# robin-karlsson0/pc-accumulation-lib

Measured on AMD Instinct MI355X. Metric: Mpoints/s projected+accumulated and BEV frames/s @256x256; 1/2/4/8 GPU, higher is better.
Workload: dtype f64; 1 GPU; KITTI-360 single forward cam, 120k pts/frame, 200 m horizon (~201 live frames, 5169634 stored pts), one 256x256x21 BEV per integrated frame; points_per_frame=120000, bev_px=256, view_m=80

## Files before the change

### include/pca.h

```cpp
#ifndef PCA_H
#define PCA_H

#include <stdint.h>

#ifdef __cplusplus
extern "C" {
#endif

#define PCA_VERSION 2

typedef struct pca_ctx pca_ctx;

typedef struct {
    double *x, *y, *z;
    float *intensity;
    uint32_t *rgbs;
    int32_t *inst;
    uint8_t *dyn;
    int64_t capacity;
    uint32_t *frame_box;
} pca_store;

#define PCA_STATUS_STORE_OVERFLOW 1u
#define PCA_STATUS_UV_OUT_OF_IMAGE 2u
// ... 322 lines not shown

typedef struct pca_host_track pca_host_track;
typedef struct {
    const void *pts;
    const void *rgb;
    const void *sem;
    const void *sem_gt;
    int32_t n;
    uint32_t host_mask;
} pca_kitti_obs;
int pca_kitti_integrate(pca_ctx *ctx, const pca_kitti_obs *obs, const double P[12], int H, int W,
                        const uint64_t filter_mask[4], const pca_store *store, int64_t *frame_off , int slot,
                        int sample_mode, pca_host_track *track, const double *T_new_prev, double horizon, int64_t *evicted,
                        double *path_length, void *stream);
void pca_host_camera_cone(const double P[12], int H, int W, double cone[15]);
int pca_host_view_hull(int F, const double *then , const float *box , const double *cone ,
                       const double now[12], const pca_bev_params *prm, int *first, int *last);
int pca_bev_bin_range(pca_ctx *ctx, int slot_first, int slot_last_plus1);
int pca_bev_view_hint(pca_ctx *ctx, int slot0, int F, const double *then, const float *box, const double *cone, const double now[12],
                      const pca_bev_params *prm);
void pca_f32_box_decode(const uint32_t *rows , int n, float *box );

int pca_debug_bev_level1(const pca_ctx *ctx, int out[4]);
int pca_debug_icp_layout(int32_t n_src, int32_t n_tgt, int64_t out[16]);

int pca_k1_defer(pca_ctx *ctx, int on);
int pca_k1_flush(pca_ctx *ctx);
int pca_kitti_generate_bev(pca_ctx *ctx, const pca_store *store, const int64_t *frame_off , int slot_begin,
                           int slot_split, int slot_end, int64_t max_points, const pca_bev_params *prm,
                           const double *pending_Ts, const int *pending_slot_ends, int n_pending, int write_back,
                           void *workspace , int64_t workspace_bytes, uint16_t *planes_f16 ,
                           void *host_planes , const pca_host_track *track, double *traj_rows,
                           int32_t *traj_start, int32_t *n_rows, void *stream);

typedef struct {
    const pca_kitti_obs *obs; const double *P; int32_t H, W; const uint64_t *filter_mask; const pca_store *store;
    int64_t *frame_off; int32_t slot, sample_mode; pca_host_track *track; const double *T_new_prev; double horizon;
    int64_t evicted; double path_length; void *stream;
} pca_kitti_integrate_args;
int pca_kitti_integrate_v(pca_ctx *ctx, pca_kitti_integrate_args *a);
typedef struct {
    const pca_store *store; const int64_t *frame_off; int32_t slot_begin, slot_split, slot_end, pad0; int64_t max_points;
    const pca_bev_params *prm; const double *pending_Ts; const int *pending_slot_ends; int32_t n_pending, write_back;
    void *workspace; int64_t workspace_bytes; uint16_t *planes_f16; void *host_planes; const pca_host_track *track;
    double *traj_rows; int32_t *traj_start; int32_t n_rows, pad1; void *stream;
    int32_t hint_slot0, hint_F; const double *hint_then; const float *hint_box; const double *hint_cone; const double *hint_now;
// ... 88 lines not shown
```

### pc-accumulation-lib_amd/csrc/pca_bev.hip

```cpp
#include "pca_bev_common.h"
#include "pca_bev_view.h"
#include "pca_k1_body.h"
#include <cstdlib>
#include <mutex>

#define NFK (2 * TCELLS)
#ifndef AB_THREADS
#define AB_THREADS 1024
#endif
#define MAX_G 512
#ifndef BIN_RUNR
#define BIN_RUNR 4
#endif
#ifndef BIN_WPE
#define BIN_WPE 4
#endif
#ifndef BIN_UNR
#define BIN_UNR 4
#endif
#ifndef BIN_REG_P
#define BIN_REG_P 12
#endif
#ifndef C_THREADS
#define C_THREADS 256
#endif
#define C_WAVES (C_THREADS / 64)
#define C_HIST_WAVES 4
#define RGB_CAP 4096
#ifndef C_SLOT_Q
#define C_SLOT_Q 4
#endif
#define CONTIG_MIN 2560
#define HEAVY_MIN_DEFAULT 2560
#define FLAG_ROAD (1u << 24)
#define FLAG_DYNOBJ (1u << 25)

struct __attribute__((aligned(16))) RecF { double z; uint32_t iw; uint32_t cw; };
struct RecD { double z; double inten; uint32_t c; uint32_t fk; };

struct alignas(16) BevArgs {
    pca_store st;
    const double *intensity64;
    const int64_t *frame_off;
    int slot_begin, slot_split, slot_end;
// ... 6 lines not shown
    int heavy_min;
    int stagger;
    uint32_t *key;
    uint32_t *bh;
    uint32_t *boff;
    int Gk;
    int bin_first, bin_end;
    int k1_slot, k1_n;
    uint32_t *bh0;
    int split;
    uint32_t *heavy_hint;
    uint32_t heavy_hint_known;
    uint32_t *span_hint;
    uint32_t span_hint_known;
    int heavy_launched;
    uint32_t *heavy;
    void *recs;
    double *planes;
    uint16_t *planes_f16;
    double *extra;
    uint32_t *status;
    int dbg;
    int band_r0, band_rows;
};
#define HQ_CLASSES 32
#define HQ_CURSOR 32
#define HQ_IDS 64

struct Window { int64_t lo, hi, sp, c_lo, c_hi; };

#define K1_SEG 4096
#define K1_RIDE 32
__device__ __forceinline__ int64_t window_end(const BevArgs &a)
{
    const int e = a.Gk ? a.k1_slot : a.slot_end;
    return a.frame_off[a.bin_end < e ? a.bin_end : e];
}
__device__ __forceinline__ int64_t window_begin(const BevArgs &a) { return a.frame_off[a.bin_first]; }
__device__ __forceinline__ Window chunk_of(const BevArgs &a, int &g)
{
    Window w;
    w.lo = window_begin(a);
    const int64_t hi0 = window_end(a);
    w.sp = (a.Gk && a.slot_split > a.k1_slot) ? hi0 : a.frame_off[a.slot_split];
    w.hi = (hi0 - w.lo > a.max_points) ? w.lo + a.max_points : hi0;
    const int G = a.G - a.Gk;
// ... 102 lines not shown
        s_dyn[threadIdx.x] = w;
    }
    BIN_STAMP(0);
    int g;
    const Window w = chunk_of(a, g);
    const int64_t chunk = seg_stride(w.hi - w.lo, a.G - a.Gk);
    const bool split = bev_split(a, w.hi - w.lo);
    const int hs = split ? 6 : 7;
    const int n_hist = split ? 2 * a.T : a.T;
    uint32_t *s_cur = s_lds + n_hist;
    if ((int)blockIdx.x == a.Gk) {
        const int64_t end_ub = a.Gk ? a.frame_off[a.k1_slot] + a.k1_n : a.frame_off[a.slot_end];
        if (threadIdx.x == 0 && end_ub - a.frame_off[a.slot_begin] > a.max_points + a.k1_n) pca_raise(a.status, PCA_STATUS_STORE_OVERFLOW);
        if (threadIdx.x < HQ_IDS) a.heavy[threadIdx.x] = 0;
        if (threadIdx.x == 0 && a.span_hint) {
            const uint32_t kp = (uint32_t)((w.hi - w.lo + 1023) >> 10);
            if (kp != a.span_hint_known) *a.span_hint = kp;
        }
    }
    for (int t = threadIdx.x; t < n_hist; t += AB_THREADS) s_h[t] = 0;
    __syncthreads();
    const PendHi pend_hi = owed_bounds(a.owed, a.frame_off, a.slot_begin, w.lo);
    const int64_t reg_hi = w.c_lo + (int64_t)REG_P * AB_THREADS < w.c_hi ? w.c_lo + (int64_t)REG_P * AB_THREADS : w.c_hi;
    uint32_t rkey[REG_P > 0 ? REG_P : 1], rrgb[REG_P > 0 ? REG_P : 1];
    float rinten[REG_P > 0 ? REG_P : 1];
    double rz[REG_P > 0 ? REG_P : 1];
    const uint32_t n_reg = w.c_lo < reg_hi ? (uint32_t)(reg_hi - w.c_lo) : 0u;
    auto rel = [&](int64_t p) -> uint32_t {
        const int64_t d = p - w.c_lo;
        return d <= 0 ? 0u : (d < (int64_t)n_reg ? (uint32_t)d : n_reg);
    };
    const uint32_t sp_rel = rel(w.sp);
    if (REG_P > 0 && n_reg > 0) {
        const double *xb = a.st.x + w.c_lo, *yb = a.st.y + w.c_lo, *zb = a.st.z + w.c_lo;
        const uint8_t *db = a.st.dyn + w.c_lo;
        const ViewConst vc = view_const(a.prm, a.tx, a.band_r0, a.band_rows);
        double XA[UNR], YA[UNR], ZA[UNR];
        uint32_t DA[UNR];
        auto issue = [&](int j0, double (&X)[UNR], double (&Y)[UNR], double (&Z)[UNR], uint32_t (&D)[UNR]) {
#pragma unroll
            for (int u = 0; u < UNR; ++u) {
                const uint32_t i = (uint32_t)(j0 + u) * AB_THREADS + threadIdx.x, ic = i < n_reg ? i : 0u;
                X[u] = xb[ic];
                Y[u] = yb[ic];
                Z[u] = zb[ic];
                D[u] = db[ic];
            }
        };
        auto work = [&](int j0, double (&X)[UNR], double (&Y)[UNR], double (&Z)[UNR], uint32_t (&D)[UNR]) {
            uint32_t n_moved = 0;
#pragma unroll 1
            for (int k = 0; k < a.owed.n_pend; ++k) {
                const Mat34 &Tk = a.owed.pend_T[k];
                const uint32_t n_owe = rel(k == 0 ? pend_hi.v[0] : k == 1 ? pend_hi.v[1] : k == 2 ? pend_hi.v[2] : pend_hi.v[3]);
                if (n_owe == 0) continue;
                n_moved = n_owe > n_moved ? n_owe : n_moved;
                const double t0 = Tk.m[0], t1 = Tk.m[1], t2 = Tk.m[2], t3 = Tk.m[3], t4 = Tk.m[4], t5 = Tk.m[5], t6 = Tk.m[6],
                             t7 = Tk.m[7], t8 = Tk.m[8], t9 = Tk.m[9], t10 = Tk.m[10], t11 = Tk.m[11];
                const uint32_t batch_end = (uint32_t)(j0 + UNR) * AB_THREADS < n_reg ? (uint32_t)(j0 + UNR) * AB_THREADS : n_reg;
                const bool all_owe = n_owe >= batch_end;
                if (all_owe) {
#pragma unroll
                    for (int u = 0; u < UNR; ++u) {
                        const double nx = fma(t2, Z[u], fma(t1, Y[u], t0 * X[u])) + t3;
                        const double ny = fma(t6, Z[u], fma(t5, Y[u], t4 * X[u])) + t7;
                        const double nz = fma(t10, Z[u], fma(t9, Y[u], t8 * X[u])) + t11;
                        X[u] = nx; Y[u] = ny; Z[u] = nz;
                    }
                } else {
#pragma unroll
                    for (int u = 0; u < UNR; ++u) {
                        const uint32_t i = (uint32_t)(j0 + u) * AB_THREADS + threadIdx.x;
                        const bool owed = i < n_owe;
                        const double nx = fma(t2, Z[u], fma(t1, Y[u], t0 * X[u])) + t3;
                        const double ny = fma(t6, Z[u], fma(t5, Y[u], t4 * X[u])) + t7;
                        const double nz = fma(t10, Z[u], fma(t9, Y[u], t8 * X[u])) + t11;
                        X[u] = owed ? nx : X[u]; Y[u] = owed ? ny : Y[u]; Z[u] = owed ? nz : Z[u];
                    }
                }
            }
            if (a.owed.write_back && n_moved > 0) {
                double *xw = a.st.x + w.c_lo, *yw = a.st.y + w.c_lo, *zw = a.st.z + w.c_lo;
#pragma unroll
                for (int u = 0; u < UNR; ++u) {
                    const uint32_t i = (uint32_t)(j0 + u) * AB_THREADS + threadIdx.x;
                    if (i < n_moved) { xw[i] = X[u]; yw[i] = Y[u]; zw[i] = Z[u]; }
                }
            }
#pragma unroll
            for (int u = 0; u < UNR; ++u) {
                const uint32_t i = (uint32_t)(j0 + u) * AB_THREADS + threadIdx.x;
                rkey[j0 + u] = view_key_lean<BAND>(vc, X[u], Y[u], Z[u], i < n_reg && D[u] != 1u, i >= sp_rel ? 1u : 0u);
                rz[j0 + u] = Z[u];
                if (rkey[j0 + u] != KEY_INVALID) atomicAdd(&s_h[rkey[j0 + u] >> hs], 1u);
            }
        };
#pragma unroll
        for (int j0 = 0; j0 < REG_P; j0 += UNR) {
            issue(j0, XA, YA, ZA, DA);
            work(j0, XA, YA, ZA, DA);
        }
    } else {
#pragma unroll
        for (int j = 0; j < REG_P; ++j) { rkey[j] = KEY_INVALID; rz[j] = 0.0; }
    }
    BIN_STAMP(1);
    constexpr int MUNR = BIN_UNR;
    const ViewConst vcm = view_const(a.prm, a.tx, a.band_r0, a.band_rows);
    for (int64_t base = reg_hi + threadIdx.x; base < w.c_hi; base += MUNR * AB_THREADS) {
        double X[MUNR], Y[MUNR], Z[MUNR];
        uint8_t D[MUNR];
#pragma unroll
        for (int u = 0; u < MUNR; ++u) {
            const int64_t p = base + u * AB_THREADS;
            const bool in = p < w.c_hi;
            X[u] = in ? a.st.x[p] : 0.0;
            Y[u] = in ? a.st.y[p] : 0.0;
            Z[u] = in ? a.st.z[p] : 0.0;
            D[u] = in ? a.st.dyn[p] : (uint8_t)1;
        }
#pragma unroll
        for (int u = 0; u < MUNR; ++u) {
            const int64_t p = base + u * AB_THREADS;
            if (p >= w.c_hi) continue;
            const BinPoint b = bin_point<BAND>(a, vcm, w, pend_hi, p, X[u], Y[u], Z[u], D[u]);
            if (b.key != KEY_INVALID) atomicAdd(&s_h[b.key >> hs], 1u);
            a.key[p - w.lo] = b.key;
        }
    }
    __syncthreads();
    BIN_STAMP(2);
    bin_scan_tables(a, s_h, s_cur, s_wsum, split, g);
// ... 1 lines not shown
    BIN_STAMP(3);
    const uint32_t seg = (uint32_t)((int64_t)a.Gk * K1_SEG + (int64_t)(g - a.Gk) * chunk);
    if (REG_P > 0 && n_reg > 0) {
        const uint32_t *cb = a.st.rgbs + w.c_lo;
        const float *ib = a.st.intensity + w.c_lo;
#pragma unroll
        for (int j = 0; j < REG_P; ++j) {
            const uint32_t i = (uint32_t)j * AB_THREADS + threadIdx.x, ic = rkey[j] != KEY_INVALID ? i : 0u;
            rrgb[j] = cb[ic];
            rinten[j] = ib[ic];
        }
        {
            uint32_t touch = 0;
#pragma unroll
            for (int j = 0; j < REG_P; ++j) touch |= rrgb[j] ^ __float_as_uint(rinten[j]);
            asm volatile("" ::"v"(touch));
        }
#pragma unroll
        for (int j = 0; j < REG_P; ++j) {
            if (rkey[j] == KEY_INVALID) continue;
            const uint32_t pos = seg + atomicAdd(&s_cur[rkey[j] >> hs], 1u);
            bin_store<I64>(a, s_dyn, pos, rkey[j], rrgb[j], rz[j], 0.0, rinten[j]);
        }
    }
    BIN_STAMP(4);
    const bool stale = a.owed.n_pend > 0 && !a.owed.write_back;
    for (int64_t base = reg_hi + threadIdx.x; base < w.c_hi; base += MUNR * AB_THREADS) {
        uint32_t key[MUNR], pos[MUNR], rgbs[MUNR];
        double zz[MUNR], iv[MUNR], xs[MUNR], ys[MUNR];
#pragma unroll
        for (int u = 0; u < MUNR; ++u) {
            const int64_t p = base + u * AB_THREADS;
            key[u] = p < w.c_hi ? a.key[p - w.lo] : KEY_INVALID;
        }
#pragma unroll
        for (int u = 0; u < MUNR; ++u) {
            const int64_t p = base + u * AB_THREADS;
            const bool ok = key[u] != KEY_INVALID;
            rgbs[u] = ok ? a.st.rgbs[p] : 0u;
            zz[u] = ok ? a.st.z[p] : 0.0;
            xs[u] = (ok && stale) ? a.st.x[p] : 0.0;
            ys[u] = (ok && stale) ? a.st.y[p] : 0.0;
            if (I64) iv[u] = ok ? a.intensity64[p] : 0.0;
            else iv[u] = ok ? (double)a.st.intensity[p] : 0.0;
        }
#pragma unroll
        for (int u = 0; u < MUNR; ++u) {
            const int64_t p = base + u * AB_THREADS;
            const bool ok = key[u] != KEY_INVALID;
            if (ok && stale) apply_owed(a.owed, pend_hi, p, xs[u], ys[u], zz[u]);
// ... 998 lines not shown
static inline int n_groups(int64_t max_points)
{
    const int max_g = max_groups(), per_g = (int)pca_env_int("PCA_BEV_CHUNK", 8192, 1024);
    int64_t g = (max_points + per_g - 1) / per_g;
    return (int)(g < 1 ? 1 : (g > max_g ? max_g : g));
}

struct BevLayout { int T, G; int64_t bh, boff, bh0, heavy, recs, total; };
static BevLayout bev_layout(int64_t max_points, int px)
{
    if (max_points < 1) max_points = 1;
    const int64_t T = (int64_t)band_rows(px) * tiles_x(px), G = n_groups(max_points);
    const int64_t table = pca_align256((G + K1_RIDE + 8) * T * 4);
    BevLayout l;
    l.T = (int)T; l.G = (int)G;
    l.bh = pca_align256(max_points * 4);
    l.boff = l.bh + table; l.bh0 = l.boff + table;
    l.heavy = l.bh0 + table;
    l.recs = l.heavy + pca_align256((HQ_IDS + HQ_CLASSES * T) * 4);
    l.total = l.recs + pca_align256((max_points + G + K1_RIDE + K1_SEG) * 24) + 512;
    return l;
}

typedef void (*BevKernel)(BevArgs);
typedef void (*BevManyKernel)();
struct BevKernelSet {
    BevKernel bin, cells, heavy[2][2];
    BevManyKernel bin_many, cells_many, heavy_many;
    int bin_lds;
};
#define K1_RIDE_LDS (80 * 1024)
#define BEV_WHOLE_SET(I)                                                                                                          \
    { bev_tile_bin<I>, bev_tile_cells<I>,                                                                                         \
      {{bev_tile_cells_heavy<I, false, false>, bev_tile_cells_heavy<I, false, true>}, {bev_tile_cells_heavy<I, true, false>, bev_tile_cells_heavy<I, true, true>}}, \
      bev_tile_bin_many<I>, bev_tile_cells_many<I>, bev_tile_cells_heavy_many<I>, 128 * 1024 }
#define BEV_BAND_SET(I)                                                                                                           \
    { bev_tile_bin_band<I>, bev_tile_cells_band<I>,                                                                               \
      {{bev_tile_cells_heavy_band<I, false>, nullptr}, {bev_tile_cells_heavy_band<I, true>, nullptr}},                           \
      bev_tile_bin_band_many<I>, bev_tile_cells_band_many<I>, bev_tile_cells_heavy_band_many<I>, BAND_TILES * 8 }
static const BevKernelSet g_bev_kernels[2][2] = {{BEV_WHOLE_SET(false), BEV_BAND_SET(false)}, {BEV_WHOLE_SET(true), BEV_BAND_SET(true)}};
#undef BEV_WHOLE_SET
#undef BEV_BAND_SET

extern "C" {

int64_t pca_bev_workspace_bytes(int64_t max_points, int px) { return bev_layout(max_points, px).total; }

int pca_bev_generate(pca_ctx *ctx, const pca_store *store, const double *intensity64, const int64_t *frame_off,
                     int slot_begin, int slot_split, int slot_end, int64_t max_points, const pca_bev_params *prm,
                     const double *pending_T, int pending_slot_end, void *workspace, int64_t workspace_bytes,
                     double *planes, uint16_t *planes_f16, void *stream)
{
    return pca_bev_generate_ex(ctx, store, intensity64, frame_off, slot_begin, slot_split, slot_end, max_points, prm,
                               pending_T, pending_slot_end, workspace, workspace_bytes, planes, planes_f16, nullptr, stream);
// ... 30 lines not shown
    const BevLayout l = bev_layout(max_points, prm->px);
    if (workspace_bytes < l.total) { ctx->err = "bev: workspace too small"; return -1; }
    a.st = *store;
    a.intensity64 = intensity64;
    a.frame_off = frame_off;
    a.slot_begin = slot_begin; a.slot_split = slot_split; a.slot_end = slot_end;
    a.max_points = max_points;
    a.prm = *prm;
    if (bev_fill_owed(ctx, "bev", pending_Ts, pending_slot_ends, n_pending, slot_begin, slot_end, a.owed)) return -1;
    a.owed.write_back = write_back ? 1 : 0;
    a.tx = tiles_x(prm->px);
    a.band_rows = band_rows(prm->px);
    a.band_r0 = 0;
    a.T = l.T;
    a.G = l.G;
    bev_table_order(a);
    char *w = reinterpret_cast<char *>(pca_align256(reinterpret_cast<intptr_t>(workspace)));
    a.key = reinterpret_cast<uint32_t *>(w);
    a.bh = reinterpret_cast<uint32_t *>(w + l.bh);
    a.boff = reinterpret_cast<uint32_t *>(w + l.boff);
    a.bh0 = reinterpret_cast<uint32_t *>(w + l.bh0);
    a.split = 0;
    a.Gk = 0; a.k1_slot = -1; a.k1_n = 0;
    a.bin_first = slot_begin; a.bin_end = slot_end;
    a.heavy = reinterpret_cast<uint32_t *>(w + l.heavy);
    a.recs = w + l.recs;
    a.planes = planes;
    a.planes_f16 = planes_f16;
    a.extra = extra_planes;
    { const int hm = (int)PCA_ENV_ONCE("PCA_BEV_HEAVY_MIN", HEAVY_MIN_DEFAULT); a.heavy_min = (hm < 1 || hm > RGB_CAP) ? RGB_CAP : hm; }
    a.dbg = (int)PCA_ENV_ONCE("PCA_BEV_DBG", 0);
    a.stagger = (int)PCA_ENV_ONCE("PCA_BEV_STAGGER", 0, 0, 64);
    a.status = ctx->ticket + 1;
    a.tile_mult = bev_tile_mult((a.tx & 3) == 0 ? a.T / 4 : a.T);
    a.heavy_hint = nullptr; a.heavy_hint_known = 0; a.heavy_launched = 1;
    a.span_hint = nullptr; a.span_hint_known = 0;
    return 0;
}

static int bev_set_lds_attributes(pca_ctx *ctx)
{
    static bool lds_set = false;
    if (lds_set) return 0;
    auto grant = [](auto k, size_t bytes) { return k ? hipFuncSetAttribute(reinterpret_cast<const void *>(k), hipFuncAttributeMaxDynamicSharedMemorySize, (int)bytes) : hipSuccess; };
    for (int i = 0; i < 4; ++i) {
        const BevKernelSet &ks = g_bev_kernels[i >> 1][i & 1];
        PCA_CHECK(ctx, grant(ks.bin, ks.bin_lds));
        PCA_CHECK(ctx, grant(ks.bin_many, ks.bin_lds));
        for (int v = 0; v < 4; ++v) PCA_CHECK(ctx, grant(ks.heavy[v >> 1][v & 1], HEAVY_LDS_BYTES));
        PCA_CHECK(ctx, grant(ks.heavy_many, HEAVY_LDS_BYTES));
    }
    PCA_CHECK(ctx, grant(bev_tile_bin_k1, K1_RIDE_LDS));
    lds_set = true;
    return 0;
}

static void bev_decide_heavy(pca_ctx *ctx, BevArgs &a, bool tuned)
{
    if (!tuned) return;
    a.heavy_hint = ctx->heavy_hint_dev;
    a.heavy_hint_known = *ctx->heavy_hint;
    if (a.heavy_hint_known != 0) ctx->heavy_cooldown = 64;
    else if (ctx->heavy_cooldown > 0) --ctx->heavy_cooldown;
    a.heavy_launched = a.heavy_hint_known != 0 || ctx->heavy_cooldown > 0;
    if (PCA_ENV_ONCE("PCA_BEV_HEAVY_ALWAYS", 0)) a.heavy_launched = 1;
}

static size_t bev_decide_split(BevArgs &a, bool tuned)
{
    const int sp = tuned ? (int)PCA_ENV_ONCE("PCA_BEV_SPLIT", 1) : 0;
    a.split = (sp && a.heavy_launched && !a.intensity64 && (size_t)a.T * 16 <= 128 * 1024) ? (sp == 2 ? 2 : 1) : 0;
    return (size_t)a.T * 8 * (a.split ? 2 : 1);
}

static int bev_decide_k1_ride(pca_ctx *ctx, const BevArgs &a, bool tuned, size_t lds, hipStream_t s, K1Args *k1a, int *nt)
{
    *nt = 0;
    if (!ctx->k1_pend.valid) return 0;
    if (!tuned) return pca_k1_flush_pending(ctx);
    const int fk = (int)PCA_ENV_ONCE("PCA_FUSE_K1", 1);
    const pca_ctx::K1Pending &pd = ctx->k1_pend;
    bool owed_ok = true;
    for (int k = 0; k < a.owed.n_pend; ++k) owed_ok = owed_ok && a.owed.pend_slot_end[k] <= pd.slot;
    const bool fuse = fk && owed_ok && !a.intensity64 && pd.stream == s && pd.slot == a.slot_end - 1 && pd.slot >= a.slot_begin &&
                      pd.frame_off == a.frame_off && pd.store.x == a.st.x && lds <= K1_RIDE_LDS && pd.fr.n <= K1_RIDE * K1_SEG &&
                      pd.fr.n <= a.max_points && pca_k1_prepare_pending(ctx, k1a, nt, s) == 0 && *nt <= K1_RIDE;
    if (PCA_ENV_ONCE("PCA_FUSE_DBG", 0) && !fuse)
        fprintf(stderr, "bev: K1 of slot %d not taken along: switch %d owed_ok %d i64 %d stream %d slot %d (window %d..%d) frame_off %d store %d lds %zu n %d max_points %lld nt %d\n",
                pd.slot, fk, (int)owed_ok, a.intensity64 != nullptr, pd.stream == s, pd.slot == a.slot_end - 1, a.slot_begin, a.slot_end,
                pd.frame_off == a.frame_off, pd.store.x == a.st.x, lds, pd.fr.n, (long long)a.max_points, *nt);
    if (fuse) return 0;
    *nt = 0;
    return pca_k1_flush_pending(ctx);
}

struct BevBinRange { bool given; int first, end; };
static int bev_decide_bin_range(pca_ctx *ctx, BevArgs &a, bool tuned, const BevBinRange &r)
{
    if (!r.given || !PCA_ENV_ONCE("PCA_BEV_CULL", 1) || (a.owed.n_pend > 0 && a.owed.write_back)) return 0;
    const int f = r.first > a.slot_begin ? r.first : a.slot_begin, e = r.end < a.slot_end ? r.end : a.slot_end;
    a.bin_first = f; a.bin_end = e < f ? f : e;
    if (!tuned) return 0;
    const int64_t pts = PCA_ENV_ONCE("PCA_BEV_ONE_ROUND_PTS", 14500);
    a.span_hint = ctx->heavy_hint_dev + 1;
    a.span_hint_known = ctx->heavy_hint[1];
    return (pts > 0 && a.span_hint_known != 0 && (int64_t)a.span_hint_known * 1024 <= pts * ctx->n_cu && a.G > ctx->n_cu) ? ctx->n_cu : 0;
}

static void bev_size_level1(pca_ctx *ctx, BevArgs &a, int nt, int one_round)
{
    if (nt == 0) { if (one_round > 0) { a.G = one_round; bev_table_order(a); } return; }
    const pca_ctx::K1Pending &pd = ctx->k1_pend;
    const int cap = max_groups(), G0 = a.G;
    if (one_round) one_round -= nt;
    a.G = one_round > 0 ? one_round + nt : (G0 + nt <= cap || (cap - 2 * nt) * 4 < 3 * G0) ? G0 + nt : cap - nt;
    a.Gk = nt; bev_table_order(a); a.k1_slot = pd.slot; a.k1_n = pd.fr.n;
    a.max_points = a.max_points - pd.fr.n;
}

static int bev_launch_raster(pca_ctx *ctx, const BevKernelSet &ks, const BevArgs &a, const K1Args *k1, size_t lds, hipStream_t s)
{
    if (k1) {
        PCA_LAUNCH_SHM(ctx, PCA_K_BEV_BIN, bev_tile_bin_k1, dim3(a.G), dim3(AB_THREADS), lds, s, a, *k1);
        pca_k1_pending_launched(ctx, s);
    } else PCA_LAUNCH_SHM(ctx, PCA_K_BEV_BIN, ks.bin, dim3(a.G), dim3(AB_THREADS), lds, s, a);
    PCA_LAUNCH(ctx, PCA_K_BEV_CELLS, ks.cells, dim3(a.T), dim3(C_THREADS), s, a);
    if (!a.heavy_launched) return 0;
    const int heavy_grid = a.T < ctx->n_cu ? a.T : ctx->n_cu;
    const BevKernel heavy = ks.heavy[a.extra != nullptr][a.split != 0];
    if (!heavy) { ctx->err = "bev: no heavy kernel for a split banded raster"; return -1; }
    PCA_LAUNCH_SHM(ctx, PCA_K_BEV_CELLS_HEAVY, heavy, dim3(heavy_grid), dim3(H_THREADS), HEAVY_LDS_BYTES, s, a);
    return 0;
}

int pca_bev_generate_chain(pca_ctx *ctx, const pca_store *store, const double *intensity64, const int64_t *frame_off,
                           int slot_begin, int slot_split, int slot_end, int64_t max_points, const pca_bev_params *prm,
                           const double *pending_Ts, const int *pending_slot_ends, int n_pending, int write_back,
                           void *workspace, int64_t workspace_bytes, double *planes, uint16_t *planes_f16,
                           double *extra_planes, void *stream)
{
    if (!ctx) return -1;
    const BevBinRange bin_range = {ctx->bin_valid, ctx->bin_first, ctx->bin_end};
    ctx->bin_valid = false;
    if (max_points < 1) max_points = 1;
    hipStream_t s = (hipStream_t)stream;
    PCA_CHECK(ctx, hipSetDevice(ctx->device));
    BevArgs a;
    if (bev_prepare(ctx, store, intensity64, frame_off, slot_begin, slot_split, slot_end, max_points, prm, pending_Ts,
                    pending_slot_ends, n_pending, write_back, workspace, workspace_bytes, planes, planes_f16, extra_planes, a))
        return -1;
    if (bev_set_lds_attributes(ctx)) return -1;
    const bool tuned = a.band_rows == a.tx;
    const BevKernelSet &ks = g_bev_kernels[intensity64 != nullptr][!tuned];
    K1Args k1a;
    int nt = 0;
    bev_decide_heavy(ctx, a, tuned);
    const size_t lds = bev_decide_split(a, tuned);
    if (bev_decide_k1_ride(ctx, a, tuned, lds, s, &k1a, &nt)) return -1;
    const int one_round = bev_decide_bin_range(ctx, a, tuned, bin_range);
    bev_size_level1(ctx, a, nt, one_round);
    ctx->last_level1[0] = a.G; ctx->last_level1[1] = a.Gk; ctx->last_level1[2] = a.bin_first; ctx->last_level1[3] = a.bin_end;
    if (ctx->profiling == 2) pca_prof_begin(ctx, PCA_K_BEV_UNIT, s);
    for (int r0 = 0, rows = a.band_rows; r0 < a.tx; r0 += rows) {
        if (!tuned) {
            bev_set_band(a, r0);
            if (r0 > 0 && a.owed.write_back) a.owed.n_pend = 0;
        }
        if (bev_launch_raster(ctx, ks, a, nt ? &k1a : nullptr, lds, s)) return -1;
    }
    if (ctx->profiling == 2) pca_prof_end(ctx, s);
    PCA_CHECK(ctx, hipGetLastError());
    return 0;
}

int pca_bev_generate_many(pca_ctx *ctx, const pca_store *store, const double *intensity64, const int64_t *frame_off,
                          const pca_bev_job *jobs, int n_jobs, int64_t max_points, void *workspace,
                          int64_t workspace_bytes, void *stream)
{
    if (!ctx) return -1;
    if (pca_k1_flush_pending(ctx)) return -1;
    ctx->bin_valid = false;
// ... 14 lines not shown
    if (up_bytes > ctx->bevm_cap) {
        if (ctx->bevm_pin) PCA_CHECK(ctx, hipHostFree(ctx->bevm_pin));
        ctx->bevm_pin = nullptr; ctx->bevm_cap = 0;
        PCA_CHECK(ctx, hipHostMalloc(&ctx->bevm_pin, (size_t)(2 * up_bytes), hipHostMallocMapped));
        ctx->bevm_cap = 2 * up_bytes;
    }
    if (!ctx->bevm_ev) PCA_CHECK(ctx, hipEventCreateWithFlags(&ctx->bevm_ev, hipEventDisableTiming));
    BevArgs *ha = reinterpret_cast<BevArgs *>(ctx->bevm_pin);
    char *ws = reinterpret_cast<char *>(pca_align256(reinterpret_cast<intptr_t>(workspace)));
    for (int k = 0; k < n_jobs; ++k) {
        const pca_bev_job &j = jobs[k];
        if (j.prm.px != px) { ctx->err = "bev: the rasters of one call share the grid size"; return -1; }
        if (bev_prepare(ctx, store, intensity64, frame_off, j.slot_begin, j.slot_split, j.slot_end, max_points, &j.prm, nullptr,
                        nullptr, 0, 1, ws + per * k, per, j.planes, j.planes_f16, nullptr, ha[k]))
            return -1;
    }
    for (int b = n_bands - 1; b >= 0 && n_bands > 1; --b)
        for (int k = 0; k < n_jobs; ++k) {
            BevArgs &d = ha[(int64_t)b * n_jobs + k];
            d = ha[k];
            bev_set_band(d, b * rows);
        }
    if (bev_set_lds_attributes(ctx)) return -1;
    const size_t lds = (size_t)l.T * 8;
    static std::mutex many_mutex;
    static hipEvent_t many_last[64] = {};
    std::lock_guard<std::mutex> many_lock(many_mutex);
    hipEvent_t &last = many_last[ctx->device & 63];
    if (last) PCA_CHECK(ctx, hipStreamWaitEvent(s, last, 0));
    else PCA_CHECK(ctx, hipEventCreateWithFlags(&last, hipEventDisableTiming));
    if (ctx->profiling) pca_prof_begin(ctx, PCA_K_BEV_UNIT, s);
    for (int b = 0; b < n_bands; ++b)
    for (int j0 = 0; j0 < n_jobs; j0 += PCA_BEV_MANY_MAX) {
        const int nk = n_jobs - j0 < PCA_BEV_MANY_MAX ? n_jobs - j0 : PCA_BEV_MANY_MAX;
        const int64_t k0 = (int64_t)b * n_jobs + j0;
        const int Tb = ha[k0].T;
        const int heavy_grid = Tb < 8 ? Tb : 8;
        static void *many_dev[64] = {};
        if (!many_dev[ctx->device & 63]) PCA_CHECK(ctx, hipGetSymbolAddress(&many_dev[ctx->device & 63], HIP_SYMBOL(g_bev_many)));
        if (pca_small_copy()) PCA_CHECK(ctx, hipMemcpyToSymbolAsync(HIP_SYMBOL(g_bev_many), ha + k0, sizeof(BevArgs) * (size_t)nk, 0, hipMemcpyHostToDevice, s));
        else if (pca_fetch_block(ctx, ha, (int64_t)sizeof(BevArgs) * k0, many_dev[ctx->device & 63], (int64_t)sizeof(BevArgs) * nk, s)) return -1;
        hipLaunchKernelGGL(ks.bin_many, dim3(l.G, nk), dim3(AB_THREADS), lds, s);
        hipLaunchKernelGGL(ks.cells_many, dim3(Tb, nk), dim3(C_THREADS), 0, s);
        hipLaunchKernelGGL(ks.heavy_many, dim3(heavy_grid, nk), dim3(H_THREADS), HEAVY_LDS_BYTES, s);
    }
    PCA_CHECK(ctx, hipEventRecord(ctx->bevm_ev, s));
    ctx->bevm_busy = true;
// ... 28 lines not shown
}

int pca_bev_warp(pca_ctx *ctx, const uint16_t *planes_f16, uint16_t *out_f16, int n_planes, int px, double a_1, double a_2,
                 double b_1, double b_2, void *stream)
{
    if (!ctx) return -1;
    if (!planes_f16 || !out_f16 || planes_f16 == out_f16 || n_planes < 1 || px < 1 || px > 65535) { ctx->err = "warp: bad arguments"; return -1; }
    if (!(a_1 == a_1 && a_2 == a_2 && b_1 == b_1 && b_2 == b_2)) { ctx->err = "warp: NaN coefficient"; return -1; }
    hipStream_t s = (hipStream_t)stream;
    PCA_CHECK(ctx, hipSetDevice(ctx->device));
    WarpArgs a;
    a.in = planes_f16; a.out = out_f16; a.n_planes = n_planes; a.px = px;
    a.a1 = a_1; a.a2 = a_2; a.b1 = b_1; a.b2 = b_2;
    hipLaunchKernelGGL(bev_warp, dim3((px + 255) / 256, px), dim3(256), 0, s, a);
    PCA_CHECK(ctx, hipGetLastError());
    return 0;
}

int pca_debug_bev_stamps(unsigned long long *out)
{
    return (int)hipMemcpyFromSymbol(out, HIP_SYMBOL(g_dbg_stamps), sizeof(unsigned long long) * 8192);
}

int pca_debug_bev_level1(const pca_ctx *ctx, int out[4])
{
    if (!ctx || !out) return -1;
    for (int k = 0; k < 4; ++k) out[k] = ctx->last_level1[k];
    return 0;
}

}
```

### pc-accumulation-lib_amd/pca_amd/_lib.py

```python
import ctypes as C
import os
import threading

import numpy as np

_HERE = os.path.dirname(os.path.abspath(__file__))
LIB_PATH = os.path.join(_HERE, 'libpca_hip.so')

STATUS_STORE_OVERFLOW = 1
STATUS_UV_OUT_OF_IMAGE = 2
STATUS_NEGATIVE_INTENSITY = 4
STATUS_LOOKBACK_TIMEOUT = 8
STATUS_LANES_BISECT_CAP = 16
SAMPLE_MODES = {'nearest': 0, 'bilinear': 1}

EXPORTS = ('pca_version', 'pca_ctx_create', 'pca_ctx_destroy', 'pca_last_error', 'pca_status', 'pca_status_peek', 'pca_status_mirror',
           'pca_kitti_project_sample_filter', 'pca_kitti_project_sample_filter_ex',
           'pca_nusc_sample_filter_transform', 'pca_nusc_sample_filter_transform_ex', 'pca_nusc_sample_filter_transform_batch', 'pca_sample_bilinear', 'pca_nusc_project_cams',
           'pca_nusc_merge_sweeps_workspace_bytes', 'pca_nusc_merge_sweeps', 'pca_retransform', 'pca_retransform_batch_tail',
           'pca_mark_dynamic',
           'pca_bev_workspace_bytes', 'pca_bev_generate', 'pca_bev_generate_ex', 'pca_bev_generate_chain', 'pca_bev_generate_many', 'pca_bev_class_workspace_bytes', 'pca_bev_class_planes', 'pca_bev_elev_workspace_bytes', 'pca_bev_elev_partition', 'pca_bev_voxel_workspace_bytes', 'pca_bev_voxel_labels', 'pca_bev_voxel_rays', 'pca_bev_carve_workspace_bytes', 'pca_bev_voxel_carve', 'pca_bev_instances_workspace_bytes', 'pca_bev_voxel_instances', 'pca_bev_instance_boxes_workspace_bytes', 'pca_bev_instance_boxes', 'pca_render_camera', 'pca_bev_voxel_camera', 'pca_voxel_pool', 'pca_voxel_pack', 'pca_voxel_distance_workspace_bytes', 'pca_voxel_distance', 'pca_voxel_instance_match_workspace_bytes', 'pca_voxel_instance_match', 'pca_bev_warp', 'pca_lanes_workspace_bytes', 'pca_lanes_transform', 'pca_lanes_to_grid', 'pca_image_to_nchw_f32', 'pca_voxel_dedup_workspace_bytes', 'pca_voxel_dedup', 'pca_icp_workspace_bytes', 'pca_icp_register', 'pca_host_ego_to_grid',
           'pca_host_gemv4_probe', 'pca_host_gemv4_mode', 'pca_host_incr_probe', 'pca_host_incr_blocks', 'pca_host_track_create', 'pca_host_track_destroy', 'pca_host_track_len', 'pca_host_track_n_segments',
           'pca_host_track_poses', 'pca_host_track_segments', 'pca_host_track_set', 'pca_host_track_transform',
           'pca_host_track_append', 'pca_host_track_push_segment', 'pca_host_track_incr', 'pca_host_track_evict_beyond',
           'pca_host_track_step', 'pca_host_track_trigger', 'pca_host_stage_h2d', 'pca_host_d2h_async', 'pca_host_d2h_wait',
           'pca_deflate_workspace_bytes', 'pca_deflate_chunks', 'pca_deflate_chunks_dyn', 'pca_host_crc32_combine', 'pca_host_gzip_assemble',
           'pca_preview_stream_bytes', 'pca_preview_workspace_bytes', 'pca_preview_sheets', 'pca_adler32_chunks', 'pca_host_adler32_combine', 'pca_host_png_assemble',
           'pca_kitti_integrate', 'pca_kitti_generate_bev', 'pca_k1_defer', 'pca_k1_flush', 'pca_host_camera_cone', 'pca_host_view_hull', 'pca_bev_bin_range', 'pca_bev_view_hint', 'pca_kitti_integrate_v', 'pca_kitti_generate_bev_v', 'pca_f32_box_decode', 'pca_debug_bev_level1', 'pca_debug_icp_layout',
           'pca_profile_enable', 'pca_profile_read')

KERNEL_IDS = ('kitti_project_sample_filter', 'nusc_sample_filter_transform', 'nusc_project_cams', 'retransform',
              'mark_dynamic', 'bev_bin', 'bev_scan', 'bev_scatter', 'bev_cells', 'bev_cells_heavy', 'voxel_dedup', 'bev_unit', 'icp', 'bev_class_bin', 'bev_class_cells', 'bev_elev_bin', 'bev_elev_cells')
KERNEL_IDS_VOXEL = ('bev_voxel_bin', 'bev_voxel_cells')
KERNEL_IDS_RAYS = ('bev_voxel_rays', )
KERNEL_IDS_RENDER = ('render_zbuffer', 'render_resolve')
KERNEL_IDS_CARVE = ('bev_carve_ends', 'bev_carve_rays', 'bev_carve_flags')
KERNEL_IDS_INST = ('bev_inst_init', 'bev_inst_merge', 'bev_inst_compress', 'bev_inst_sums', 'bev_inst_offsets', 'bev_inst_number',
                   'bev_inst_write', 'bev_inst_points')
KERNEL_IDS_CAMERA = ('bev_camera_rays', )
KERNEL_IDS_SSC = ('voxel_pool', 'voxel_pack')
KERNEL_IDS_DIST = ('voxel_dist_lines', 'voxel_dist_rows')
KERNEL_IDS_BOX = ('bev_box_table', 'bev_box_count', 'bev_box_offsets', 'bev_box_scatter', 'bev_box_extents', 'bev_box_near',
                  'bev_box_choose')
BEV_INST_COLS = 9
BOX_CRITERIA = {'area': 0, 'edge': 1}
DYN_MODES = {'static': 0, 'all': 1, 'dynamic': 2}
BEV_EXTRA_PLANES = ('elevation_max', 'elevation_mean', 'intensity_mean')


class PcaStore(C.Structure):
    _fields_ = [('x', C.c_void_p), ('y', C.c_void_p), ('z', C.c_void_p), ('intensity', C.c_void_p),
# ... 264 lines not shown
    lib.pca_preview_stream_bytes.argtypes = [i32]
    lib.pca_preview_stream_bytes.restype = i64
    lib.pca_preview_workspace_bytes.argtypes = [i32, i32]
    lib.pca_preview_workspace_bytes.restype = i64
    lib.pca_preview_sheets.argtypes = [vp, vp, i32, i32, vp, i64, vp, i32, vp, vp, i32, vp, vp, vp]
    lib.pca_adler32_chunks.argtypes = [vp, vp, vp, i64, vp, vp]
    lib.pca_host_adler32_combine.argtypes = [C.c_uint32, C.c_uint32, i64]
    lib.pca_host_adler32_combine.restype = C.c_uint32
    lib.pca_host_png_assemble.argtypes = [i32, i32, i32, vp, vp, C.c_uint32, vp, i64]
    lib.pca_host_png_assemble.restype = i64
    lib.pca_kitti_integrate.argtypes = [vp, C.POINTER(PcaKittiObs), C.POINTER(C.c_double), i32, i32, C.POINTER(C.c_uint64),
                                        C.POINTER(PcaStore), vp, i32, i32, vp, vp, C.c_double, C.POINTER(C.c_int64),
                                        C.POINTER(C.c_double), vp]
    lib.pca_kitti_generate_bev.argtypes = [vp, C.POINTER(PcaStore), vp, i32, i32, i32, i64, C.POINTER(PcaBevParams), vp, vp,
                                           i32, i32, vp, i64, vp, vp, vp, vp, vp, C.POINTER(C.c_int32), vp]
    lib.pca_host_camera_cone.argtypes = [vp, i32, i32, vp]
    lib.pca_host_camera_cone.restype = None
    lib.pca_host_view_hull.argtypes = [i32, vp, vp, vp, vp, vp, C.POINTER(C.c_int), C.POINTER(C.c_int)]
    lib.pca_bev_bin_range.argtypes = [vp, i32, i32]
    lib.pca_bev_view_hint.argtypes = [vp, i32, i32, vp, vp, vp, vp, vp]
    lib.pca_f32_box_decode.argtypes = [vp, i32, vp]
    lib.pca_f32_box_decode.restype = None
    lib.pca_debug_bev_level1.argtypes = [vp, vp]
    lib.pca_debug_icp_layout.argtypes = [i32, i32, C.POINTER(C.c_int64)]
    lib.pca_kitti_integrate_v.argtypes = [vp, vp]
    lib.pca_kitti_generate_bev_v.argtypes = [vp, vp]
    lib.pca_k1_defer.argtypes = [vp, i32]
    lib.pca_k1_flush.argtypes = [vp]
    lib.pca_profile_enable.argtypes = [vp, i32]
    lib.pca_profile_read.argtypes = [vp, i32, C.POINTER(C.c_double), C.POINTER(C.c_int64)]
    _lib = lib
    return lib


class Context:

    _by_device = {}
    _raw_stream = None
    _tls = threading.local()

    def __init__(self, device_index):
        import torch
        if not torch.cuda.is_available():
            raise RuntimeError('pca_amd needs an AMD GPU (torch.cuda.is_available() is False); '
                               'there is no CPU fallback')
        self.lib = load()
# ... 119 lines not shown
```

Measured before the change: 1556 Mpoints/s.

## Park extra binned points' keys and z in LDS to avoid re-reading them

Extends the bin kernel's resident-point window beyond the register-held points by parking the keys and z values of up to BIN_LDS_P extra rows per thread in dynamic LDS during the histogram pass. The scatter pass reads them back instead of re-reading x/y/z from global memory and recomputing the view key. LDS grants are raised up to the per-CU limit, and the feature turns off when the intensity64 path is used or there is not enough room. The larger LDS footprint can lower occupancy, and it adds a debug query for the chosen parking depth.

```diff
diff --git a/include/pca.h b/include/pca.h
--- a/include/pca.h
+++ b/include/pca.h
@@ -368,6 +368,7 @@
 void pca_f32_box_decode(const uint32_t *rows , int n, float *box );
 
 int pca_debug_bev_level1(const pca_ctx *ctx, int out[4]);
+int pca_debug_bev_lds(int out[2]);
 int pca_debug_icp_layout(int32_t n_src, int32_t n_tgt, int64_t out[16]);
 
 int pca_k1_defer(pca_ctx *ctx, int on);
diff --git a/pc-accumulation-lib_amd/csrc/pca_bev.hip b/pc-accumulation-lib_amd/csrc/pca_bev.hip
--- a/pc-accumulation-lib_amd/csrc/pca_bev.hip
+++ b/pc-accumulation-lib_amd/csrc/pca_bev.hip
@@ -20,6 +20,12 @@
 #endif
 #ifndef BIN_REG_P
 #define BIN_REG_P 12
+#endif
+#ifndef BIN_LDS_P
+#define BIN_LDS_P 4
+#endif
+#ifndef BIN_LUNR
+#define BIN_LUNR 2
 #endif
 #ifndef C_THREADS
 #define C_THREADS 256
@@ -72,6 +78,7 @@
     uint32_t *status;
     int dbg;
     int band_r0, band_rows;
+    int lds_p;
 };
 #define HQ_CLASSES 32
 #define HQ_CURSOR 32
@@ -220,14 +227,21 @@
     __syncthreads();
     const PendHi pend_hi = owed_bounds(a.owed, a.frame_off, a.slot_begin, w.lo);
     const int64_t reg_hi = w.c_lo + (int64_t)REG_P * AB_THREADS < w.c_hi ? w.c_lo + (int64_t)REG_P * AB_THREADS : w.c_hi;
+    const int lds_p = REG_P > 0 ? a.lds_p : 0;
+    const int64_t res_cap = (int64_t)(REG_P + lds_p) * AB_THREADS;
+    const int64_t res_hi = w.c_lo + res_cap < w.c_hi ? w.c_lo + res_cap : w.c_hi;
+    double *s_pz = reinterpret_cast<double *>(s_lds + 2 * n_hist);
+    uint32_t *s_pk = reinterpret_cast<uint32_t *>(s_pz + lds_p * AB_THREADS);
     uint32_t rkey[REG_P > 0 ? REG_P : 1], rrgb[REG_P > 0 ? REG_P : 1];
     float rinten[REG_P > 0 ? REG_P : 1];
     double rz[REG_P > 0 ? REG_P : 1];
     const uint32_t n_reg = w.c_lo < reg_hi ? (uint32_t)(reg_hi - w.c_lo) : 0u;
+    const uint32_t n_res = w.c_lo < res_hi ? (uint32_t)(res_hi - w.c_lo) : 0u;
     auto rel = [&](int64_t p) -> uint32_t {
         const int64_t d = p - w.c_lo;
-        return d <= 0 ? 0u : (d < (int64_t)n_reg ? (uint32_t)d : n_reg);
+        return d <= 0 ? 0u : (d < (int64_t)n_res ? (uint32_t)d : n_res);
     };
+    const int n_park_rows = (int)((n_res - n_reg + AB_THREADS - 1) / AB_THREADS);
     const uint32_t sp_rel = rel(w.sp);
     if (REG_P > 0 && n_reg > 0) {
         const double *xb = a.st.x + w.c_lo, *yb = a.st.y + w.c_lo, *zb = a.st.z + w.c_lo;
@@ -235,17 +249,19 @@
         const ViewConst vc = view_const(a.prm, a.tx, a.band_r0, a.band_rows);
         double XA[UNR], YA[UNR], ZA[UNR];
         uint32_t DA[UNR];
-        auto issue = [&](int j0, double (&X)[UNR], double (&Y)[UNR], double (&Z)[UNR], uint32_t (&D)[UNR]) {
-#pragma unroll
-            for (int u = 0; u < UNR; ++u) {
-                const uint32_t i = (uint32_t)(j0 + u) * AB_THREADS + threadIdx.x, ic = i < n_reg ? i : 0u;
+        auto issue = [&](int j0, auto &X, auto &Y, auto &Z, auto &D) {
+            constexpr int N = (int)(sizeof(D) / sizeof(D[0]));
+#pragma unroll
+            for (int u = 0; u < N; ++u) {
+                const uint32_t i = (uint32_t)(j0 + u) * AB_THREADS + threadIdx.x, ic = i < n_res ? i : 0u;
                 X[u] = xb[ic];
                 Y[u] = yb[ic];
                 Z[u] = zb[ic];
                 D[u] = db[ic];
             }
         };
-        auto work = [&](int j0, double (&X)[UNR], double (&Y)[UNR], double (&Z)[UNR], uint32_t (&D)[UNR]) {
+        auto work = [&](int j0, auto &X, auto &Y, auto &Z, auto &D, auto &&keep) {
+            constexpr int N = (int)(sizeof(D) / sizeof(D[0]));
             uint32_t n_moved = 0;
 #pragma unroll 1
             for (int k = 0; k < a.owed.n_pend; ++k) {
@@ -255,11 +271,11 @@
                 n_moved = n_owe > n_moved ? n_owe : n_moved;
                 const double t0 = Tk.m[0], t1 = Tk.m[1], t2 = Tk.m[2], t3 = Tk.m[3], t4 = Tk.m[4], t5 = Tk.m[5], t6 = Tk.m[6],
                              t7 = Tk.m[7], t8 = Tk.m[8], t9 = Tk.m[9], t10 = Tk.m[10], t11 = Tk.m[11];
-                const uint32_t batch_end = (uint32_t)(j0 + UNR) * AB_THREADS < n_reg ? (uint32_t)(j0 + UNR) * AB_THREADS : n_reg;
+                const uint32_t batch_end = (uint32_t)(j0 + N) * AB_THREADS < n_res ? (uint32_t)(j0 + N) * AB_THREADS : n_res;
                 const bool all_owe = n_owe >= batch_end;
                 if (all_owe) {
 #pragma unroll
-                    for (int u = 0; u < UNR; ++u) {
+                    for (int u = 0; u < N; ++u) {
                         const double nx = fma(t2, Z[u], fma(t1, Y[u], t0 * X[u])) + t3;
                         const double ny = fma(t6, Z[u], fma(t5, Y[u], t4 * X[u])) + t7;
                         const double nz = fma(t10, Z[u], fma(t9, Y[u], t8 * X[u])) + t11;
@@ -267,7 +283,7 @@
                     }
                 } else {
 #pragma unroll
-                    for (int u = 0; u < UNR; ++u) {
+                    for (int u = 0; u < N; ++u) {
                         const uint32_t i = (uint32_t)(j0 + u) * AB_THREADS + threadIdx.x;
                         const bool owed = i < n_owe;
                         const double nx = fma(t2, Z[u], fma(t1, Y[u], t0 * X[u])) + t3;
@@ -280,23 +296,35 @@
             if (a.owed.write_back && n_moved > 0) {
                 double *xw = a.st.x + w.c_lo, *yw = a.st.y + w.c_lo, *zw = a.st.z + w.c_lo;
 #pragma unroll
-                for (int u = 0; u < UNR; ++u) {
+                for (int u = 0; u < N; ++u) {
                     const uint32_t i = (uint32_t)(j0 + u) * AB_THREADS + threadIdx.x;
                     if (i < n_moved) { xw[i] = X[u]; yw[i] = Y[u]; zw[i] = Z[u]; }
                 }
             }
 #pragma unroll
-            for (int u = 0; u < UNR; ++u) {
+            for (int u = 0; u < N; ++u) {
                 const uint32_t i = (uint32_t)(j0 + u) * AB_THREADS + threadIdx.x;
-                rkey[j0 + u] = view_key_lean<BAND>(vc, X[u], Y[u], Z[u], i < n_reg && D[u] != 1u, i >= sp_rel ? 1u : 0u);
-                rz[j0 + u] = Z[u];
-                if (rkey[j0 + u] != KEY_INVALID) atomicAdd(&s_h[rkey[j0 + u] >> hs], 1u);
+                const uint32_t key = view_key_lean<BAND>(vc, X[u], Y[u], Z[u], i < n_res && D[u] != 1u, i >= sp_rel ? 1u : 0u);
+                keep(u, key, Z[u]);
+                if (key != KEY_INVALID) atomicAdd(&s_h[key >> hs], 1u);
             }
         };
 #pragma unroll
         for (int j0 = 0; j0 < REG_P; j0 += UNR) {
             issue(j0, XA, YA, ZA, DA);
-            work(j0, XA, YA, ZA, DA);
+            work(j0, XA, YA, ZA, DA, [&](int u, uint32_t key, double z) { rkey[j0 + u] = key; rz[j0 + u] = z; });
+        }
+        if (n_park_rows > 0) {
+            double XL[BIN_LUNR], YL[BIN_LUNR], ZL[BIN_LUNR];
+            uint32_t DL[BIN_LUNR];
+#pragma unroll
+            for (int jl = 0; jl < BIN_LDS_P; jl += BIN_LUNR) {
+                if (jl >= n_park_rows) break;
+                issue(REG_P + jl, XL, YL, ZL, DL);
+                work(REG_P + jl, XL, YL, ZL, DL, [&](int u, uint32_t key, double z) {
+                    if (jl + u < lds_p) { s_pk[(jl + u) * AB_THREADS + threadIdx.x] = key; s_pz[(jl + u) * AB_THREADS + threadIdx.x] = z; }
+                });
+            }
         }
     } else {
 #pragma unroll
@@ -305,7 +333,7 @@
     BIN_STAMP(1);
     constexpr int MUNR = BIN_UNR;
     const ViewConst vcm = view_const(a.prm, a.tx, a.band_r0, a.band_rows);
-    for (int64_t base = reg_hi + threadIdx.x; base < w.c_hi; base += MUNR * AB_THREADS) {
+    for (int64_t base = res_hi + threadIdx.x; base < w.c_hi; base += MUNR * AB_THREADS) {
         double X[MUNR], Y[MUNR], Z[MUNR];
         uint8_t D[MUNR];
 #pragma unroll
@@ -353,10 +381,33 @@
             const uint32_t pos = seg + atomicAdd(&s_cur[rkey[j] >> hs], 1u);
             bin_store<I64>(a, s_dyn, pos, rkey[j], rrgb[j], rz[j], 0.0, rinten[j]);
         }
+        if (n_park_rows > 0) {
+            constexpr int LP = BIN_LDS_P < REG_P ? BIN_LDS_P : REG_P;
+#pragma unroll
+            for (int j = 0; j < LP; ++j) {
+                rkey[j] = s_pk[(j < n_park_rows ? j : 0) * AB_THREADS + threadIdx.x];
+                if (j >= n_park_rows) rkey[j] = KEY_INVALID;
+                const uint32_t i = (uint32_t)(REG_P + j) * AB_THREADS + threadIdx.x, ic = rkey[j] != KEY_INVALID ? i : 0u;
+                rrgb[j] = cb[ic];
+                rinten[j] = ib[ic];
+            }
+            {
+                uint32_t touch = 0;
+#pragma unroll
+                for (int j = 0; j < LP; ++j) touch |= rrgb[j] ^ __float_as_uint(rinten[j]);
+                asm volatile("" ::"v"(touch));
+            }
+#pragma unroll
+            for (int j = 0; j < LP; ++j) {
+                if (rkey[j] == KEY_INVALID) continue;
+                const uint32_t pos = seg + atomicAdd(&s_cur[rkey[j] >> hs], 1u);
+                bin_store<I64>(a, s_dyn, pos, rkey[j], rrgb[j], s_pz[j * AB_THREADS + threadIdx.x], 0.0, rinten[j]);
+            }
+        }
     }
     BIN_STAMP(4);
     const bool stale = a.owed.n_pend > 0 && !a.owed.write_back;
-    for (int64_t base = reg_hi + threadIdx.x; base < w.c_hi; base += MUNR * AB_THREADS) {
+    for (int64_t base = res_hi + threadIdx.x; base < w.c_hi; base += MUNR * AB_THREADS) {
         uint32_t key[MUNR], pos[MUNR], rgbs[MUNR];
         double zz[MUNR], iv[MUNR], xs[MUNR], ys[MUNR];
 #pragma unroll
@@ -1401,6 +1452,7 @@
     return l;
 }
 
+static int g_last_lds[2] = {0, 0};
 typedef void (*BevKernel)(BevArgs);
 typedef void (*BevManyKernel)();
 struct BevKernelSet {
@@ -1409,6 +1461,12 @@
     int bin_lds;
 };
 #define K1_RIDE_LDS (80 * 1024)
+#define LDS_CU (160 * 1024)
+#define BIN_STATIC_LDS 256
+#define K1_RIDE_STATIC_LDS 74240
+#define BIN_PARK_BYTES(lds_p) ((size_t)(lds_p) * AB_THREADS * 12)
+static_assert(BIN_LDS_P >= 0 && BIN_LDS_P <= BIN_REG_P, "pass B handles the parked points in the register points' registers");
+static_assert(K1_RIDE_LDS <= LDS_CU - K1_RIDE_STATIC_LDS, "a riding K1's static LDS and the largest histogram share a CU");
 #define BEV_WHOLE_SET(I)                                                                                                          \
     { bev_tile_bin<I>, bev_tile_cells<I>,                                                                                         \
       {{bev_tile_cells_heavy<I, false, false>, bev_tile_cells_heavy<I, false, true>}, {bev_tile_cells_heavy<I, true, false>, bev_tile_cells_heavy<I, true, true>}}, \
@@ -1485,6 +1543,7 @@
     a.bh0 = reinterpret_cast<uint32_t *>(w + l.bh0);
     a.split = 0;
     a.Gk = 0; a.k1_slot = -1; a.k1_n = 0;
+    a.lds_p = 0;
     a.bin_first = slot_begin; a.bin_end = slot_end;
     a.heavy = reinterpret_cast<uint32_t *>(w + l.heavy);
     a.recs = w + l.recs;
@@ -1508,12 +1567,13 @@
     auto grant = [](auto k, size_t bytes) { return k ? hipFuncSetAttribute(reinterpret_cast<const void *>(k), hipFuncAttributeMaxDynamicSharedMemorySize, (int)bytes) : hipSuccess; };
     for (int i = 0; i < 4; ++i) {
         const BevKernelSet &ks = g_bev_kernels[i >> 1][i & 1];
-        PCA_CHECK(ctx, grant(ks.bin, ks.bin_lds));
-        PCA_CHECK(ctx, grant(ks.bin_many, ks.bin_lds));
+        const size_t room = LDS_CU - BIN_STATIC_LDS, most = ks.bin_lds + BIN_PARK_BYTES(BIN_LDS_P);
+        PCA_CHECK(ctx, grant(ks.bin, most < room ? most : room));
+        PCA_CHECK(ctx, grant(ks.bin_many, most < room ? most : room));
         for (int v = 0; v < 4; ++v) PCA_CHECK(ctx, grant(ks.heavy[v >> 1][v & 1], HEAVY_LDS_BYTES));
         PCA_CHECK(ctx, grant(ks.heavy_many, HEAVY_LDS_BYTES));
     }
-    PCA_CHECK(ctx, grant(bev_tile_bin_k1, K1_RIDE_LDS));
+    PCA_CHECK(ctx, grant(bev_tile_bin_k1, LDS_CU - K1_RIDE_STATIC_LDS));
     lds_set = true;
     return 0;
 }
@@ -1557,6 +1617,13 @@
     return pca_k1_flush_pending(ctx);
 }
 
+static int bev_decide_lds_p(const void *intensity64, size_t lds, bool k1_rides)
+{
+    if (intensity64 || BIN_LDS_P == 0 || !PCA_ENV_ONCE("PCA_BEV_LDS_P", 1)) return 0;
+    const size_t fixed = k1_rides ? K1_RIDE_STATIC_LDS : BIN_STATIC_LDS;
+    return fixed + lds + BIN_PARK_BYTES(BIN_LDS_P) <= LDS_CU ? BIN_LDS_P : 0;
+}
+
 struct BevBinRange { bool given; int first, end; };
 static int bev_decide_bin_range(pca_ctx *ctx, BevArgs &a, bool tuned, const BevBinRange &r)
 {
@@ -1583,6 +1650,7 @@
 
 static int bev_launch_raster(pca_ctx *ctx, const BevKernelSet &ks, const BevArgs &a, const K1Args *k1, size_t lds, hipStream_t s)
 {
+    lds += BIN_PARK_BYTES(a.lds_p);
     if (k1) {
         PCA_LAUNCH_SHM(ctx, PCA_K_BEV_BIN, bev_tile_bin_k1, dim3(a.G), dim3(AB_THREADS), lds, s, a, *k1);
         pca_k1_pending_launched(ctx, s);
@@ -1620,6 +1688,8 @@
     bev_decide_heavy(ctx, a, tuned);
     const size_t lds = bev_decide_split(a, tuned);
     if (bev_decide_k1_ride(ctx, a, tuned, lds, s, &k1a, &nt)) return -1;
+    a.lds_p = bev_decide_lds_p(intensity64, lds, nt > 0);
+    g_last_lds[0] = a.lds_p; g_last_lds[1] = (int)(lds + BIN_PARK_BYTES(a.lds_p));
     const int one_round = bev_decide_bin_range(ctx, a, tuned, bin_range);
     bev_size_level1(ctx, a, nt, one_round);
     ctx->last_level1[0] = a.G; ctx->last_level1[1] = a.Gk; ctx->last_level1[2] = a.bin_first; ctx->last_level1[3] = a.bin_end;
@@ -1680,7 +1750,9 @@
             bev_set_band(d, b * rows);
         }
     if (bev_set_lds_attributes(ctx)) return -1;
-    const size_t lds = (size_t)l.T * 8;
+    const int lds_p = bev_decide_lds_p(intensity64, (size_t)l.T * 8, false);
+    for (int64_t k = 0; k < (int64_t)n_jobs * n_bands; ++k) ha[k].lds_p = lds_p;
+    const size_t lds = (size_t)l.T * 8 + BIN_PARK_BYTES(lds_p);
     static std::mutex many_mutex;
     static hipEvent_t many_last[64] = {};
     std::lock_guard<std::mutex> many_lock(many_mutex);
@@ -1755,6 +1827,13 @@
     return (int)hipMemcpyFromSymbol(out, HIP_SYMBOL(g_dbg_stamps), sizeof(unsigned long long) * 8192);
 }
 
+int pca_debug_bev_lds(int out[2])
+{
+    if (!out) return -1;
+    out[0] = g_last_lds[0]; out[1] = g_last_lds[1];
+    return 0;
+}
+
 int pca_debug_bev_level1(const pca_ctx *ctx, int out[4])
 {
     if (!ctx || !out) return -1;
diff --git a/pc-accumulation-lib_amd/pca_amd/_lib.py b/pc-accumulation-lib_amd/pca_amd/_lib.py
--- a/pc-accumulation-lib_amd/pca_amd/_lib.py
+++ b/pc-accumulation-lib_amd/pca_amd/_lib.py
@@ -26,7 +26,7 @@
            'pca_host_track_step', 'pca_host_track_trigger', 'pca_host_stage_h2d', 'pca_host_d2h_async', 'pca_host_d2h_wait',
            'pca_deflate_workspace_bytes', 'pca_deflate_chunks', 'pca_deflate_chunks_dyn', 'pca_host_crc32_combine', 'pca_host_gzip_assemble',
            'pca_preview_stream_bytes', 'pca_preview_workspace_bytes', 'pca_preview_sheets', 'pca_adler32_chunks', 'pca_host_adler32_combine', 'pca_host_png_assemble',
-           'pca_kitti_integrate', 'pca_kitti_generate_bev', 'pca_k1_defer', 'pca_k1_flush', 'pca_host_camera_cone', 'pca_host_view_hull', 'pca_bev_bin_range', 'pca_bev_view_hint', 'pca_kitti_integrate_v', 'pca_kitti_generate_bev_v', 'pca_f32_box_decode', 'pca_debug_bev_level1', 'pca_debug_icp_layout',
+           'pca_kitti_integrate', 'pca_kitti_generate_bev', 'pca_k1_defer', 'pca_k1_flush', 'pca_host_camera_cone', 'pca_host_view_hull', 'pca_bev_bin_range', 'pca_bev_view_hint', 'pca_kitti_integrate_v', 'pca_kitti_generate_bev_v', 'pca_f32_box_decode', 'pca_debug_bev_level1', 'pca_debug_bev_lds', 'pca_debug_icp_layout',
            'pca_profile_enable', 'pca_profile_read')
 
 KERNEL_IDS = ('kitti_project_sample_filter', 'nusc_sample_filter_transform', 'nusc_project_cams', 'retransform',
@@ -337,6 +337,7 @@
     lib.pca_f32_box_decode.argtypes = [vp, i32, vp]
     lib.pca_f32_box_decode.restype = None
     lib.pca_debug_bev_level1.argtypes = [vp, vp]
+    lib.pca_debug_bev_lds.argtypes = [vp]
     lib.pca_debug_icp_layout.argtypes = [i32, i32, C.POINTER(C.c_int64)]
     lib.pca_kitti_integrate_v.argtypes = [vp, vp]
     lib.pca_kitti_generate_bev_v.argtypes = [vp, vp]
```

Result: faster. 1577 Mpoints/s, median of 6 (+1.3%).
